# YuyangSunshine/ABR_IOD

Hardware: AMD Instinct MI355X
Metric: training images/sec (R50-C4 Faster R-CNN + ARD) (higher is better)
Workload: dtype f32 (tensors, accumulation and error bound; contractions via a 2-term fp16 split of both operands scaled by their amax, 3 cross products on the fp16 matrix cores: f16x3)

## Files before the change

abr_iod_amd/csrc/common.h:

```cpp
#pragma once
#include <hip/hip_runtime.h>
#include <stdint.h>
#include <stdio.h>

#include <functional>
#include <vector>

#include "abr_iod_hip.h"

namespace abr {

__device__ __forceinline__ float relu_f(const float v) { return v < 0.f ? 0.f : v; }


void set_error(const char* fmt, ...);

#define ABR_REQUIRE(cond, ...)                 \
    do {                                       \
        if (!(cond)) {                         \
            ::abr::set_error(__VA_ARGS__);     \
            return ABR_E_INVALID;              \
        }                                      \
    } while (0)

// ... 9 lines not shown
constexpr int kWave = 64;
constexpr int kNumXCD = 8;

__device__ __forceinline__ unsigned xcd_remap(unsigned bid, unsigned nblk) {
    const unsigned q = nblk / kNumXCD, r = nblk % kNumXCD;
    const unsigned xcd = bid % kNumXCD, pos = bid / kNumXCD;
    const unsigned base = xcd < r ? xcd * (q + 1) : r * (q + 1) + (xcd - r) * q;
    return base + pos;
}

__device__ __forceinline__ float wave_sum(float v) {
#pragma unroll
    for (int o = 32; o > 0; o >>= 1) v += __shfl_xor(v, o, 64);
    return v;
}
__device__ __forceinline__ float wave_max(float v) {
#pragma unroll
    for (int o = 32; o > 0; o >>= 1) v = fmaxf(v, __shfl_xor(v, o, 64));
    return v;
}

template <int NW>
__device__ __forceinline__ float block_sum(float v, float* sm) {
    v = wave_sum(v);
    const int w = threadIdx.x >> 6, l = threadIdx.x & 63;
    __syncthreads();
    if (l == 0) sm[w] = v;
    __syncthreads();
    float t = 0.f;
#pragma unroll
    for (int i = 0; i < NW; i++) t += sm[i];
    return t;
}

struct DetWs {
    float* part;
    unsigned* ticket;
};
DetWs det_ws(hipStream_t st, size_t nfloats);
template <int NV>
__device__ __forceinline__ bool det_sum_last(const float (&vals)[NV], const DetWs ws, float (&total)[NV]) {
    __shared__ int s_last;
    __shared__ float s_w[16];
    const unsigned nblk = gridDim.x * gridDim.y, bid = blockIdx.y * gridDim.x + blockIdx.x;
    if (threadIdx.x == 0) {
#pragma unroll
        for (int j = 0; j < NV; j++) __hip_atomic_store(ws.part + (size_t)bid * NV + j, vals[j], __ATOMIC_RELAXED, __HIP_MEMORY_SCOPE_AGENT);
        __builtin_amdgcn_fence(__ATOMIC_RELEASE, "agent");
        asm volatile("s_waitcnt vmcnt(0)" ::: "memory");
        s_last = atomicAdd(ws.ticket, 1u) == nblk - 1u;
    }
    __syncthreads();
    if (!s_last) return false;
    if (threadIdx.x == 0) {
        __builtin_amdgcn_fence(__ATOMIC_ACQUIRE, "agent");
        *ws.ticket = 0u;
    }
    __syncthreads();
#pragma unroll
    for (int j = 0; j < NV; j++) {
        float a = 0.f;
        for (unsigned i = threadIdx.x; i < nblk; i += blockDim.x) a += __hip_atomic_load(ws.part + (size_t)i * NV + j, __ATOMIC_RELAXED, __HIP_MEMORY_SCOPE_AGENT);
        a = wave_sum(a);
        __syncthreads();
        if ((threadIdx.x & 63) == 0) s_w[threadIdx.x >> 6] = a;
        __syncthreads();
        float t = 0.f;
        for (unsigned w = 0; w < (blockDim.x >> 6); w++) t += s_w[w];
        total[j] = t;
    }
    return true;
}

enum ProfId { PROF_IGEMM_128x128 = 0, PROF_IGEMM_128x64, PROF_IGEMM_64x64, PROF_IGEMM_SMALLC, PROF_WGRAD, PROF_ROIALIGN_FWD,
              PROF_ROIALIGN_BWD, PROF_IGEMM_BF16, PROF_WGRAD_BF16,
              PROF_X6_128x128, PROF_X6_128x64, PROF_X6_64x64, PROF_X6W_128x128, PROF_X6W_128x64, PROF_X6W_64x64, PROF_X6W_TAIL64,
              PROF_H3W_128x128, PROF_H3W_128x64, PROF_H3W_64x64, PROF_WGRAD_H3,
              PROF_F16W_128x128, PROF_F16W_128x64, PROF_F16W_64x64, PROF_WGRAD_F16, PROF_COUNT };
struct AmaxRef;
int wino_input_transform(const float* x, int B, int H, int W, int C, float* V, hipStream_t st, const AmaxRef* amax = nullptr);
int wino_output_transform(const float* M, int B, int H, int W, int N, const float* scale, const float* bias, int relu, const float* mask,
                          float* out, hipStream_t st, const AmaxRef* amax = nullptr);
int wino_outgrad_transform(const float* gy, int B, int H, int W, int N, float* Mg, hipStream_t st, const AmaxRef* amax = nullptr);
int wino_wgrad_inverse(const float* dU, int N, int C, const float* scale, float* dw, hipStream_t st);
float* wino_ws(hipStream_t st, size_t floats);
enum DerivedKind { DERIVED_NONE = -1, DERIVED_WINO_U = 0, DERIVED_X6_PLANES = 1, DERIVED_WINO_U_X6_PLANES = 2, DERIVED_H3_PLANES = 3, DERIVED_WINO_U_H3_PLANES = 4 };
void* derived_cached(const void* w, int kind, size_t bytes, int64_t version, hipStream_t st, const std::function<int(void*)>& fill);
void* derived_acquire(const void* w, int kind, size_t bytes, int64_t version, hipStream_t st, void** token, std::vector<hipStream_t>* waited = nullptr);
void derived_commit(void* const* tokens, int n, hipStream_t st);
void derived_abandon(void* const* tokens, int n);

struct ConvRoute {
    int math;
    int wgrad_math;
    bool fwd_wino;
    bool wgrad_wino;
    int64_t v_floats;
    int kind;
    int64_t rows;
    int K;
    size_t bytes;
};
ConvRoute conv_route(const abr_conv_desc& d);

struct PrepJob {
    const float* src;
    const float* scale;
    void* dst;
    int a, b, c;
    int gx, gy;
    int first_block;
};
struct PrepTable { const PrepJob* jobs; int njobs; };
template <int PrepJob::*F = &PrepJob::first_block>
__device__ __forceinline__ PrepJob prep_job(const PrepTable& t, int block) {
    int lo = 0, hi = t.njobs - 1;
    while (lo < hi) {
        const int mid = (lo + hi + 1) >> 1;
        if (t.jobs[mid].*F <= block) lo = mid; else hi = mid - 1;
    }
    return t.jobs[lo];
}
template <int PrepJob::*F = &PrepJob::first_block>
__device__ __forceinline__ PrepJob prep_job(const PrepJob& j, int) { return j; }
struct PrepJobs { int n = 0; PrepJob one{}; const PrepJob* dev = nullptr; };
template <class F>
void prep_each(const PrepJobs& s, F&& f) {
    if (s.n == 1) f(s.one);
    else if (s.n > 1) f(PrepTable{s.dev, s.n});
}
__device__ __forceinline__ size_t h3_planes_bytes_dev(int rows, int K) { return (size_t)((rows + 31) / 32 * 32) * (size_t)K * 4; }
__host__ __device__ __forceinline__ int prep_transpose_tile(int Cout, int Cin, const void* w, const void* wt) {
    return (((Cout | Cin) & 3) == 0 && ((reinterpret_cast<uintptr_t>(w) | reinterpret_cast<uintptr_t>(wt)) & 15) == 0) ? 64 : 32;
}
void prep_wino_u(const PrepJobs& jobs, int blocks, hipStream_t st);
void prep_wino_h3_direct(const PrepJobs& jobs, int pack_blocks, int scale_blocks, unsigned* flags, hipStream_t st);
void derived_cache_clear();
void derived_cache_drop_range(const void* base, size_t bytes);
size_t derived_cache_bytes();

unsigned* x6_flags_ptr();
constexpr unsigned kX6TinyB = (17u << 24) - 1u;
__device__ __forceinline__ void x6_report(unsigned bmin, float nonfin, unsigned* flags) {
    unsigned f = 0;
    if (bmin < kX6TinyB) f |= ABR_X6_FLAG_TINY;
    if (nonfin != nonfin) f |= ABR_X6_FLAG_NONFINITE;
    if (f) atomicOr(flags, f);
}

struct AmaxRef {
    unsigned long long* word;
    unsigned epoch;
};
constexpr unsigned kH3RangeBinades = 18;
AmaxRef h3_amax_alloc();
int h3_amax_reduce(const float* x, int64_t n, AmaxRef ref, hipStream_t st);
void h3_amax_remember(const void* tensor, AmaxRef ref);
AmaxRef h3_amax_recall(const void* tensor);

__device__ __forceinline__ unsigned h3_amax_load(const unsigned long long* word, unsigned epoch) {
    const unsigned long long v = __hip_atomic_load(word, __ATOMIC_RELAXED, __HIP_MEMORY_SCOPE_AGENT);
    return (unsigned)(v >> 32) == epoch ? (unsigned)v : 0xFFFFFFFFu;
}
__device__ __forceinline__ void h3_scales(unsigned amax_bits, float& s, float& inv_s) {
    int e = (int)(amax_bits >> 23);
    if (amax_bits == 0u || e >= 255) { s = 1.f; inv_s = 1.f; return; }
    e = e < 15 ? 15 : e;
// ... 84 lines not shown
```

abr_iod_amd/csrc/conv_wgrad.hip:

```cpp
#include <algorithm>

#include <map>
#include <mutex>

#include "common.h"

namespace {

typedef float f32x16 __attribute__((ext_vector_type(16)));
typedef _Float16 f16x8 __attribute__((ext_vector_type(8)));

constexpr int TN_ = 128;
constexpr int TK_ = 128;
constexpr int MR = 32;

struct FastDiv {
    unsigned mul, shr, d;
    __host__ void init(unsigned div) {
        d = div;
        shr = 0;
        while ((1u << shr) < div) shr++;
        mul = (unsigned)((((unsigned long long)1 << 32) * (((unsigned long long)1 << shr) - div)) / div + 1);
    }
    __device__ __forceinline__ void divmod(unsigned n, unsigned& q, unsigned& r) const {
        q = (__umulhi(n, mul) + n) >> shr;
        r = n - q * d;
    }
};

struct WgP {
    unsigned long long* prof_ts;
    int B, H, W, Cin, Cout, R, S, stride, pad, Ho, Wo;
    int M, K;
    int tiles_n, tiles_k, splits, mt_per_split;
    int plain;
    FastDiv d_howo, d_wo;
    const float* scale;
    unsigned x_bytes, gy_bytes;
    int overwrite;
    int nbatch, tiles_pb;
    long x_bs, gy_bs, dw_bs;
    int math;
    unsigned* x6_flags;
    float* ws;
    int final_store;
    int map4;
    const unsigned long long* gy_amax;
    const unsigned long long* x_amax;
    unsigned gy_epoch, x_epoch;
    unsigned long long* h3_stats;
};

__device__ __forceinline__ float2 wg_operand_scale(const WgP& p) {
    if (!p.gy_amax) return make_float2(1.f, 1.f);
    float sg, ig, sx, ix;
    abr::h3_scales(abr::h3_amax_load(p.gy_amax, p.gy_epoch), sg, ig);
    abr::h3_scales(abr::h3_amax_load(p.x_amax, p.x_epoch), sx, ix);
    return make_float2(sg, sx);
}

typedef f32x16 wg_f32x16;

constexpr unsigned kPartBytes = 16u * 256u * 16u;

__device__ __forceinline__ void wgrad_store_tile(const WgP& p, const float (&v)[4], int tm, int tn, int c, int n0, int k0, int wm, int wn, int l31, int lh,
                                                 bool store, float* __restrict__ dw, const float2 osc = make_float2(1.f, 1.f)) {
    const int k = p.map4 ? k0 + 4 * l31 + 2 * wn + tn : k0 + wn * 64 + 2 * l31 + tn;
    if (k >= p.K) return;
#pragma unroll
    for (int e = 0; e < 4; e++) {
        const int r = 4 * c + e;
        const int i = (r & 3) + 8 * (r >> 2) + 4 * lh;
        const int n = p.map4 ? n0 + 4 * i + 2 * wm + tm : n0 + wm * 64 + 2 * i + tm;
        if (n >= p.Cout) continue;
        const float sc = (p.scale ? p.scale[n] : 1.f) * fmaxf(osc.x, osc.y);
        const float val = (v[e] * fminf(osc.x, osc.y)) * sc;
        if (store) dw[(size_t)n * p.K + k] = val;
        else unsafeAtomicAdd(dw + (size_t)n * p.K + k, val);
    }
}

__device__ __forceinline__ void wgrad_finish(const WgP& p, f32x16 (&acc)[2][2], int n0, int k0, int wm, int wn, int l31, int lh, int tid,
                                             int gtile, int split, float* __restrict__ dw) {
    if (p.ws) {
        float4* dst = reinterpret_cast<float4*>(reinterpret_cast<char*>(p.ws) + ((size_t)gtile * p.splits + split) * kPartBytes) + tid;
#pragma unroll
        for (int t = 0; t < 4; t++)
#pragma unroll
            for (int c = 0; c < 4; c++) {
                const f32x16& a = acc[t >> 1][t & 1];
                dst[(t * 4 + c) * 256] = make_float4(a[4 * c], a[4 * c + 1], a[4 * c + 2], a[4 * c + 3]);
            }
        return;
    }
    const float2 osc = wg_operand_scale(p);
#pragma unroll
    for (int t = 0; t < 4; t++)
#pragma unroll
        for (int c = 0; c < 4; c++) {
            const f32x16& a = acc[t >> 1][t & 1];
            const float v[4] = {a[4 * c], a[4 * c + 1], a[4 * c + 2], a[4 * c + 3]};
            wgrad_store_tile(p, v, t >> 1, t & 1, c, n0, k0, wm, wn, l31, lh, p.overwrite != 0, dw, osc);
        }
}

__global__ __launch_bounds__(256) void wgrad_reduce_kernel(const WgP p, float* __restrict__ dw_) {
    const int gtile = blockIdx.x >> 4, quad = blockIdx.x & 15;
    const int tid = threadIdx.x, lane = tid & 63, wave = tid >> 6;
    const float4* src = reinterpret_cast<const float4*>(reinterpret_cast<const char*>(p.ws) + (size_t)gtile * p.splits * kPartBytes) + quad * 256 + tid;
    float4 sum = make_float4(0.f, 0.f, 0.f, 0.f);
    int q = 0;
    for (; q + 4 <= p.splits; q += 4) {
        const float4 v0 = src[(size_t)q * (kPartBytes / 16)], v1 = src[(size_t)(q + 1) * (kPartBytes / 16)];
        const float4 v2 = src[(size_t)(q + 2) * (kPartBytes / 16)], v3 = src[(size_t)(q + 3) * (kPartBytes / 16)];
        sum.x += v0.x; sum.y += v0.y; sum.z += v0.z; sum.w += v0.w;
        sum.x += v1.x; sum.y += v1.y; sum.z += v1.z; sum.w += v1.w;
        sum.x += v2.x; sum.y += v2.y; sum.z += v2.z; sum.w += v2.w;
        sum.x += v3.x; sum.y += v3.y; sum.z += v3.z; sum.w += v3.w;
    }
    for (; q < p.splits; q++) {
        const float4 v = src[(size_t)q * (kPartBytes / 16)];
        sum.x += v.x; sum.y += v.y; sum.z += v.z; sum.w += v.w;
    }
    float* dw = dw_;
    int tile = gtile;
    if (p.nbatch > 1) {
        const int bt = tile / p.tiles_pb;
        tile -= bt * p.tiles_pb;
        dw += bt * p.dw_bs;
    }
    const int n0 = (tile % p.tiles_n) * TN_, k0 = (tile / p.tiles_n) * TK_;
    const float v[4] = {sum.x, sum.y, sum.z, sum.w};
    const int t = quad >> 2, c = quad & 3;
    wgrad_store_tile(p, v, t >> 1, t & 1, c, n0, k0, wave >> 1, wave & 1, lane & 31, lane >> 5, p.final_store != 0, dw, wg_operand_scale(p));
}

template <bool SB>
__global__ __launch_bounds__(256) void conv_wgrad_kernel(const WgP p, const float* __restrict__ x_,
                                                          const float* __restrict__ gy_, float* __restrict__ dw_) {
    const float* x = x_;
    const float* gy = gy_;
    float* dw = dw_;
    extern __shared__ __attribute__((aligned(16))) float smem[];
    static_assert(SB, "single-buffered only");
    abr::prof_stamp_begin(p.prof_ts);
    float* Gs = smem;
    float* As = smem + MR * TN_;

    const unsigned bid = abr::xcd_remap(blockIdx.x, gridDim.x);
    const int total_tiles = p.tiles_pb * (p.nbatch > 1 ? p.nbatch : 1);
    const int split = bid / total_tiles;
    int tile = bid % total_tiles;
    const int gtile = tile;
    if (p.nbatch > 1) {
        const int bt = tile / p.tiles_pb;
        tile -= bt * p.tiles_pb;
        x += bt * p.x_bs; gy += bt * p.gy_bs; dw += bt * p.dw_bs;
    }
    const int tile_n = tile % p.tiles_n, tile_k = tile / p.tiles_n;
    const int n0 = tile_n * TN_, k0 = tile_k * TK_;
    const int tid = threadIdx.x, lane = tid & 63, wave = tid >> 6;
    const int wm = wave >> 1, wn = wave & 1;

    const int q = tid & 31, r8 = tid >> 5;
    const int gn = n0 + q * 4;
    const bool g_ok = gn < p.Cout;
    const int ak = k0 + q * 4;
    const bool k_ok = ak < p.K;
    int fr = 0, fs = 0, fc = 0;
    if (k_ok) {
        const int rs = ak / p.Cin;
        fc = ak % p.Cin;
        fr = rs / p.S;
        fs = rs % p.S;
    }
    const int mt0 = split * p.mt_per_split;
    const int mt1 = min(mt0 + p.mt_per_split, (p.M + MR - 1) / MR);

    constexpr unsigned kOOB = 0x80000000u;
    const __amdgpu_buffer_rsrc_t rgy = __builtin_amdgcn_make_buffer_rsrc(const_cast<float*>(gy), 0, p.gy_bytes, 0x00020000);
    const __amdgpu_buffer_rsrc_t rxx = __builtin_amdgcn_make_buffer_rsrc(const_cast<float*>(x), 0, p.x_bytes, 0x00020000);
    const unsigned g_voff = g_ok ? (unsigned)(r8 * p.Cout + gn) * 4u : kOOB;
    const unsigned a_voff_plain = k_ok ? (unsigned)(r8 * p.Cin + fc) * 4u : kOOB;
    const int a_const = ((fr - p.pad) * p.W + (fs - p.pad)) * p.Cin + fc;
    float4 rg[4], ra[4];
    auto fetch = [&](__amdgpu_buffer_rsrc_t r, unsigned voff, int soff) -> float4 {
        typedef unsigned u32x4 __attribute__((ext_vector_type(4)));
        const u32x4 v = __builtin_amdgcn_raw_buffer_load_b128(r, (int)voff, soff, 0);
        return make_float4(__uint_as_float(v.x), __uint_as_float(v.y), __uint_as_float(v.z), __uint_as_float(v.w));
    };
    auto load_tile = [&](int mt) {
#pragma unroll
        for (int i = 0; i < 4; i++) {
            const int mrow = mt * MR + 8 * i;
            rg[i] = fetch(rgy, g_voff + (unsigned)(mrow * p.Cout) * 4u, 0);
            if (p.plain) {
                ra[i] = fetch(rxx, a_voff_plain + (unsigned)(mrow * p.Cin) * 4u, 0);
            } else {
                const int m = mrow + r8;
                unsigned b, rem, ho, wo;
                p.d_howo.divmod((unsigned)m, b, rem);
                p.d_wo.divmod(rem, ho, wo);
                const int hi = (int)ho * p.stride - p.pad + fr, wi = (int)wo * p.stride - p.pad + fs;
                const bool ok = k_ok & (m < p.M) & ((unsigned)hi < (unsigned)p.H) & ((unsigned)wi < (unsigned)p.W);
                const int off = (((int)b * p.H + (int)ho * p.stride) * p.W + (int)wo * p.stride) * p.Cin + a_const;
                ra[i] = fetch(rxx, ok ? (unsigned)off * 4u : kOOB, 0);
            }
        }
    };
    auto store_tile = [&]() {
#pragma unroll
        for (int i = 0; i < 4; i++) {
            *reinterpret_cast<float4*>(Gs + (r8 + 8 * i) * TN_ + q * 4) = rg[i];
            *reinterpret_cast<float4*>(As + (r8 + 8 * i) * TK_ + q * 4) = ra[i];
        }
    };

// ... 195 lines not shown
                *reinterpret_cast<u32x4*>(st_base + j * 128 + PL) = o1;
                *reinterpret_cast<u32x4*>(st_base + j * 128 + 2 * PL) = o2;
            }
        }
    };

    f32x16 acc[2][2];
#pragma unroll
    for (int i = 0; i < 2; i++)
#pragma unroll
        for (int j = 0; j < 2; j++)
#pragma unroll
            for (int r = 0; r < 16; r++) acc[i][j][r] = 0.f;

    const int l31 = lane & 31, lh = lane >> 5;
    const unsigned* const g_rd = Gs + ((lh * 4 + 2 * wm) * 32 + l31) * 4;
    const unsigned* const a_rd = As + ((lh * 4 + 2 * wn) * 32 + l31) * 4;
    auto compute_tile = [&]() {
#pragma unroll
        for (int s = 0; s < MRX / 16; s++) {
            bf16x8 G[2][NPL], A[2][NPL];
#pragma unroll
            for (int pl = 0; pl < NPL; pl++)
#pragma unroll
                for (int t = 0; t < 2; t++) {
                    G[t][pl] = *reinterpret_cast<const bf16x8*>(g_rd + pl * PL + (s * 8 + t) * 128);
                    A[t][pl] = *reinterpret_cast<const bf16x8*>(a_rd + pl * PL + (s * 8 + t) * 128);
                }
            constexpr int pg[6] = {NP == 1 ? 0 : (H3 ? 1 : 2), 0, H3 ? 0 : 1, 1, 0, 0}, pa[6] = {0, NP == 1 ? 0 : (H3 ? 1 : 2), H3 ? 0 : 1, 0, 1, 0};
#pragma unroll
            for (int t = 0; t < NP; t++)
#pragma unroll
                for (int i = 0; i < 2; i++)
#pragma unroll
                    for (int j = 0; j < 2; j++) {
                        if constexpr (HF) acc[i][j] = __builtin_amdgcn_mfma_f32_32x32x16_f16(__builtin_bit_cast(f16x8, G[i][pg[t]]), __builtin_bit_cast(f16x8, A[j][pa[t]]), acc[i][j], 0, 0, 0);
                        else acc[i][j] = __builtin_amdgcn_mfma_f32_32x32x16_bf16(G[i][pg[t]], A[j][pa[t]], acc[i][j], 0, 0, 0);
                    }
        }
    };
    if (mt0 < mt1) {
        load_tile(mt0);
        store_tile();
        __syncthreads();
        int mt = mt0;
        for (; mt + 1 < mt1; mt++) {
            load_tile(mt + 1);
            __builtin_amdgcn_sched_barrier(0);
            compute_tile();
            __syncthreads();
            store_tile();
            __syncthreads();
        }
        compute_tile();
    }
    if constexpr (HF) {
        if (chk) abr::h3_report(op_bits, nsmall, p.x6_flags, p.h3_stats);
    } else {
        if (chk) abr::x6_report(bmin, nonfin, p.x6_flags);
    }

    wgrad_finish(p, acc, n0, k0, wm, wn, l31, lh, tid, gtile, split, dw);
    abr::prof_stamp_end(p.prof_ts);
}

}

static float* wgrad_scratch(hipStream_t st, size_t units) {
    struct Ws { float* ws = nullptr; size_t units = 0; };
    static std::map<hipStream_t, Ws> pool;
    static std::mutex mu;
    std::lock_guard<std::mutex> g(mu);
    Ws& w = pool[st];
    if (w.units < units) {
        if (w.ws) { (void)hipStreamSynchronize(st); (void)hipFree(w.ws); w.ws = nullptr; w.units = 0; }
        if (hipMalloc(&w.ws, units * 65536) != hipSuccess) return nullptr;
        w.units = units;
    }
    return w.ws;
}

static void wgrad_plan_reduction(WgP& p, int tiles, hipStream_t st) {
    p.ws = nullptr;
    if (p.splits <= 1) { if (p.final_store) p.overwrite = 1; return; }
    p.ws = wgrad_scratch(st, (size_t)tiles * p.splits);
}

static void wgrad_reduce(const WgP& p, int tiles, float* dw, hipStream_t st) {
    if (p.ws) wgrad_reduce_kernel<<<(unsigned)tiles * 16u, 256, 0, st>>>(p, dw);
}

static void launch_wgrad(WgP p, const float* x, const float* gy, float* dw, void* stream) {
    const int nb = p.nbatch > 1 ? p.nbatch : 1;
    p.tiles_pb = p.tiles_n * p.tiles_k;
    const int m_tiles = (p.M + MR - 1) / MR;
    int32_t info[3];
    const int cus = abr_device_info(info) == ABR_OK ? info[0] : 256;
    const int tiles = p.tiles_n * p.tiles_k * nb;
    const int max_splits = std::max(1, (m_tiles + 7) / 8);
    int splits = 1;
    double best = -1.0;
    for (int sp = 1; sp <= max_splits; sp++) {
        const long wgs = (long)tiles * sp;
        if (wgs > 8L * cus && sp > 1) break;
        const long rounds = (wgs + cus - 1) / cus;
        double eff = (double)wgs / (double)(rounds * cus);
        if (wgs < cus) eff *= 0.5;
        else if (wgs < 2L * cus && m_tiles / (2 * sp) >= 64) eff *= 0.85;
        eff -= 0.0002 * sp;
        if (eff > best) { best = eff; splits = sp; }
    }
    if (p.overwrite) splits = 1;
    p.splits = splits;
    p.mt_per_split = (m_tiles + splits - 1) / splits;
    wgrad_plan_reduction(p, tiles, abr::as_stream(stream));
    if (p.final_store && splits > 1 && !p.ws) {
        (void)hipMemsetAsync(dw, 0, sizeof(float) * (size_t)nb * p.Cout * p.K, abr::as_stream(stream));
        p.final_store = 0;
    }
    if (p.math == ABR_MATH_BF16X6 || p.math == ABR_MATH_BF16 || p.math == ABR_MATH_F16X3 || p.math == ABR_MATH_F16) {
        static bool attr6 = false;
        const bool one = p.math == ABR_MATH_BF16;
        const bool h3 = p.math == ABR_MATH_F16X3;
        const bool f16 = p.math == ABR_MATH_F16;
        const size_t lds6 = sizeof(unsigned) * (one || f16 ? 1 : (h3 ? 2 : 3)) * (MRX / 2) * (TN_ + TK_);
        if (!attr6) {
            (void)hipFuncSetAttribute(reinterpret_cast<const void*>(conv_wgrad_x6_kernel<6>), hipFuncAttributeMaxDynamicSharedMemorySize,
                                      (int)(sizeof(unsigned) * 3 * (MRX / 2) * (TN_ + TK_)));
            attr6 = true;
        }
        p.map4 = 1;
        p.x6_flags = !one ? abr::x6_flags_ptr() : nullptr;
        p.h3_stats = (h3 && p.x6_flags) ? abr::h3_stats_ptr() : nullptr;
        if (p.h3_stats) abr::h3_stats_inspected((double)nb * p.M * ((double)p.Cout + (double)p.K));
        const int pid6 = h3 ? abr::PROF_WGRAD_H3 : (f16 ? abr::PROF_WGRAD_F16 : abr::PROF_WGRAD_BF16);
        const int rec6 = abr::prof_start(abr::as_stream(stream), pid6, 2.0 * (double)p.M * (double)p.Cout * (double)p.K * nb);
        p.prof_ts = abr::prof_clock_slot(rec6);
        abr::prof_add_bytes(pid6, 4.0 * nb * ((double)p.M * p.Cout + (p.plain ? (double)p.M * p.K : (double)p.B * p.H * p.W * p.Cin) + (double)p.Cout * p.K));
        if (h3) conv_wgrad_x6_kernel<3><<<(unsigned)(tiles * splits), 256, lds6, abr::as_stream(stream)>>>(p, x, gy, dw);
        else if (f16) conv_wgrad_x6_kernel<1, true><<<(unsigned)(tiles * splits), 256, lds6, abr::as_stream(stream)>>>(p, x, gy, dw);
        else if (one) conv_wgrad_x6_kernel<1><<<(unsigned)(tiles * splits), 256, lds6, abr::as_stream(stream)>>>(p, x, gy, dw);
        else conv_wgrad_x6_kernel<6><<<(unsigned)(tiles * splits), 256, lds6, abr::as_stream(stream)>>>(p, x, gy, dw);
        abr::prof_stop(abr::as_stream(stream), rec6);
        wgrad_reduce(p, tiles, dw, abr::as_stream(stream));
        return;
    }
    const int rec = abr::prof_start(abr::as_stream(stream), abr::PROF_WGRAD, 2.0 * (double)p.M * (double)p.Cout * (double)p.K * nb);
    p.prof_ts = abr::prof_clock_slot(rec);
    conv_wgrad_kernel<true><<<(unsigned)(tiles * splits), 256, sizeof(float) * MR * (TN_ + TK_), abr::as_stream(stream)>>>(p, x, gy, dw);
    abr::prof_stop(abr::as_stream(stream), rec);
    wgrad_reduce(p, tiles, dw, abr::as_stream(stream));
}

extern "C" int abr_conv_wgrad(const abr_conv_desc* d, const float* x, const float* gy, float* dw, void* stream) {
    ABR_REQUIRE(d && x && gy && dw, "conv_wgrad: null pointer");
    ABR_REQUIRE(d->Cin % 4 == 0 && d->Cout % 4 == 0, "conv_wgrad: Cin and Cout must be multiples of 4");
    ABR_REQUIRE(d->Ho == (d->H + 2 * d->pad - d->R) / d->stride + 1 && d->Wo == (d->W + 2 * d->pad - d->S) / d->stride + 1,
                "conv_wgrad: Ho/Wo inconsistent");
    WgP p;
    p.B = d->B; p.H = d->H; p.W = d->W; p.Cin = d->Cin; p.Cout = d->Cout; p.R = d->R; p.S = d->S;
    p.stride = d->stride; p.pad = d->pad; p.Ho = d->Ho; p.Wo = d->Wo;
    p.M = d->B * d->Ho * d->Wo;
    p.K = d->R * d->S * d->Cin;
    p.plain = (d->R == 1 && d->S == 1 && d->stride == 1 && d->pad == 0);
    p.scale = d->scale;
    const int64_t xb = (int64_t)d->B * d->H * d->W * d->Cin * 4, gb = (int64_t)p.M * d->Cout * 4;
    ABR_REQUIRE(xb < (int64_t)0x7FFFFFF0 && gb < (int64_t)0x7FFFFFF0, "conv_wgrad: activation / gradient tensors must be < 2 GB (32-bit buffer offsets)");
    p.x_bytes = (unsigned)xb; p.gy_bytes = (unsigned)gb;
    p.d_howo.init((unsigned)(d->Ho * d->Wo)); p.d_wo.init((unsigned)d->Wo);
    p.tiles_n = (p.Cout + TN_ - 1) / TN_;
    p.tiles_k = (p.K + TK_ - 1) / TK_;
    if (p.M == 0) return ABR_OK;
    p.nbatch = 1; p.tiles_pb = 0; p.x_bs = p.gy_bs = p.dw_bs = 0; p.overwrite = 0;
    p.ws = nullptr; p.final_store = 0; p.map4 = 0;
    p.x6_flags = nullptr;
    p.gy_amax = p.x_amax = nullptr; p.gy_epoch = p.x_epoch = 0; p.h3_stats = nullptr;
    hipStream_t st = abr::as_stream(stream);
    ABR_REQUIRE(d->math == ABR_MATH_F32 || d->math == ABR_MATH_BF16 || d->math == ABR_MATH_BF16X6 || d->math == ABR_MATH_F16X3 || d->math == ABR_MATH_F16,
                "conv_wgrad: unknown math mode");
    const abr::ConvRoute route = abr::conv_route(*d);
    p.math = route.wgrad_math;
    const bool h3 = p.math == ABR_MATH_F16X3 || p.math == ABR_MATH_F16;
    abr::AmaxRef gy_ref{reinterpret_cast<unsigned long long*>(const_cast<uint64_t*>(d->gy_amax)), d->gy_amax_epoch};
    abr::AmaxRef x_ref{reinterpret_cast<unsigned long long*>(const_cast<uint64_t*>(d->x_amax)), d->x_amax_epoch};
    auto need_ref = [&](abr::AmaxRef& r, const float* t, int64_t n) -> bool {
        if (r.word) return true;
        r = abr::h3_amax_alloc();
        return r.word && abr::h3_amax_reduce(t, n, r, st) == 0;
    };
    if (route.wgrad_wino) {
        const int th_n = (d->H + 3) / 4, tw_n = (d->W + 3) / 4;
        const int64_t T = (int64_t)d->B * th_n * tw_n;
        const size_t nV = (size_t)36 * T * d->Cin, nM = (size_t)36 * T * d->Cout, nU = (size_t)36 * d->Cout * d->Cin;
        float* vin = route.v_floats ? d->wino_v : nullptr;
        float* ws = abr::wino_ws(st, (vin ? 0 : nV) + nM + nU);
        if (ws) {
            float* V = vin ? vin : ws;
            float *Mg = ws + (vin ? 0 : nV), *dU = Mg + nM;
            abr::AmaxRef v_ref{nullptr, 0}, m_ref{nullptr, 0};
            if (h3) {
                if (vin) v_ref = abr::h3_amax_recall(vin);
                else v_ref = abr::h3_amax_alloc();
                m_ref = abr::h3_amax_alloc();
                ABR_REQUIRE(m_ref.word && (vin || v_ref.word), "conv_wgrad (f16x3): no amax words");
                if (vin && !v_ref.word) ABR_REQUIRE(need_ref(v_ref, vin, (int64_t)nV), "conv_wgrad (f16x3): amax reduction failed");
            }
            int bad = vin ? 0 : abr::wino_input_transform(x, d->B, d->H, d->W, d->Cin, V, st, h3 ? &v_ref : nullptr);
            bad |= abr::wino_outgrad_transform(gy, d->B, d->H, d->W, d->Cout, Mg, st, h3 ? &m_ref : nullptr);
            int32_t info[3];
            const int cus_ = abr_device_info(info) == ABR_OK ? info[0] : 256;
            const long out_tiles = 36L * ((d->Cout + TN_ - 1) / TN_) * ((d->Cin + TK_ - 1) / TK_);
            const int own = out_tiles >= 2L * cus_;
            if (!bad) {
                WgP g = p;
                g.overwrite = own;
                g.final_store = !own;
                g.B = (int)T; g.H = g.W = 1; g.R = g.S = 1; g.stride = 1; g.pad = 0; g.Ho = g.Wo = 1;
                g.M = (int)T; g.K = d->Cin; g.plain = 1; g.scale = nullptr;
                g.d_howo.init(1u); g.d_wo.init(1u);
                g.tiles_n = (g.Cout + TN_ - 1) / TN_; g.tiles_k = (g.K + TK_ - 1) / TK_;
                g.x_bytes = (unsigned)(T * d->Cin * 4); g.gy_bytes = (unsigned)(T * d->Cout * 4);
                g.nbatch = 36; g.x_bs = (long)T * d->Cin; g.gy_bs = (long)T * d->Cout; g.dw_bs = (long)d->Cout * d->Cin;
                if (h3) { g.x_amax = v_ref.word; g.x_epoch = v_ref.epoch; g.gy_amax = m_ref.word; g.gy_epoch = m_ref.epoch; }
                launch_wgrad(g, V, Mg, dU, stream);
                bad = abr::wino_wgrad_inverse(dU, d->Cout, d->Cin, d->scale, dw, st);
            }
            ABR_REQUIRE(!bad, "conv_wgrad: winograd launch failed");
            ABR_CHECK_LAUNCH("conv_wgrad (winograd)");
            return ABR_OK;
        }
    }
    if (h3) {
        ABR_REQUIRE(need_ref(gy_ref, gy, (int64_t)p.M * d->Cout) && need_ref(x_ref, x, (int64_t)d->B * d->H * d->W * d->Cin), "conv_wgrad (f16x3): amax reduction failed");
        p.gy_amax = gy_ref.word; p.gy_epoch = gy_ref.epoch; p.x_amax = x_ref.word; p.x_epoch = x_ref.epoch;
    }
    launch_wgrad(p, x, gy, dw, stream);
    ABR_CHECK_LAUNCH("conv_wgrad");
    return ABR_OK;
}
```

abr_iod_amd/csrc/conv_winograd.hip:

```cpp
#include <map>

#include <algorithm>
#include <map>
#include <functional>
#include <mutex>
#include <utility>
#include <type_traits>
#include <vector>

#include "common.h"

namespace {

template <int V>
struct vf {
    float v[V];
};
template <int V>
__device__ __forceinline__ vf<V> operator+(vf<V> a, vf<V> b) {
    vf<V> r;
#pragma unroll
    for (int i = 0; i < V; i++) r.v[i] = a.v[i] + b.v[i];
    return r;
}
// ... 323 lines not shown
#pragma unroll
                for (int j = 0; j < 4; j++) {
                    const int oy = 4 * th + i, ox = 4 * tw + j;
                    const bool in = oy < H && ox < W;
                    mk[i][j] = vld<V>(mask + (((int64_t)b * H + (in ? oy : 4 * th)) * W + (in ? ox : 4 * tw)) * N + n);
                }
        }
#pragma unroll
        for (int i = 0; i < 4; i++) {
            f2 y[4];
            at4(tcol[i][0], tcol[i][1], tcol[i][2], tcol[i][3], tcol[i][4], tcol[i][5], y[0], y[1], y[2], y[3]);
            const int oy = 4 * th + i;
            if (oy >= H) continue;
#pragma unroll
            for (int j = 0; j < 4; j++) {
                const int ox = 4 * tw + j;
                if (ox >= W) continue;
                const int64_t o = (((int64_t)b * H + oy) * W + ox) * N + n;
                f2 v;
#pragma unroll
                for (int e = 0; e < V; e++) {
                    v.v[e] = y[j].v[e] * sc.v[e] + bi.v[e];
                    if (relu) v.v[e] = abr::relu_f(v.v[e]);
                }
                if (mask) {
#pragma unroll
                    for (int e = 0; e < V; e++) v.v[e] = mk[i][j].v[e] > 0.f ? v.v[e] : 0.f;
                }
                vst(out + o, v);
                if (amax) am = vabs_max(am, v);
            }
        }
    }
    if (amax) abr::h3_amax_emit(amax, epoch, am);
}

template <typename T>
__device__ __forceinline__ void a6(const T y0, const T y1, const T y2, const T y3, T& o0, T& o1, T& o2, T& o3, T& o4, T& o5) {
    o0 = y0;
    o1 = y0 + y1 + y2 + y3;
    o2 = y0 - y1 + y2 - y3;
    o3 = y0 + 2.f * y1 + 4.f * y2 + 8.f * y3;
    o4 = y0 - 2.f * y1 + 4.f * y2 - 8.f * y3;
    o5 = y3;
}

template <int V>
__global__ __launch_bounds__(256) void wino_outgrad_kernel(const float* __restrict__ gy, int B, int H, int W, int N, int th_n, int tw_n,
                                                           float* __restrict__ Mg, unsigned long long* amax, unsigned epoch) {
    typedef vf<V> f2;
    unsigned am = 0;
    const int64_t T = (int64_t)B * th_n * tw_n;
    const int N2 = N / V;
    const int64_t total = T * N2;
    const int64_t ps = T * N;
    for (int64_t idx = (int64_t)blockIdx.x * blockDim.x + threadIdx.x; idx < total; idx += (int64_t)gridDim.x * blockDim.x) {
        const int n = V * (int)(idx % N2);
        const int64_t t = idx / N2;
        const int tw = (int)(t % tw_n), th = (int)((t / tw_n) % th_n), b = (int)(t / ((int64_t)tw_n * th_n));
        f2 tcol[6][4];
#pragma unroll
        for (int j = 0; j < 4; j++) {
            const int ox = 4 * tw + j;
            f2 y[4];
#pragma unroll
            for (int i = 0; i < 4; i++) {
                const int oy = 4 * th + i;
                y[i] = (oy < H && ox < W) ? vld<V>(gy + (((int64_t)b * H + oy) * W + ox) * N + n) : vzero<V>();
            }
            a6(y[0], y[1], y[2], y[3], tcol[0][j], tcol[1][j], tcol[2][j], tcol[3][j], tcol[4][j], tcol[5][j]);
        }
#pragma unroll
        for (int i = 0; i < 6; i++) {
            f2 v0, v1, v2, v3, v4, v5;
            a6(tcol[i][0], tcol[i][1], tcol[i][2], tcol[i][3], v0, v1, v2, v3, v4, v5);
            float* o = Mg + ((int64_t)(6 * i) * T + t) * N + n;
            vst(o, v0); vst(o + ps, v1); vst(o + 2 * ps, v2); vst(o + 3 * ps, v3); vst(o + 4 * ps, v4); vst(o + 5 * ps, v5);
            if (amax) am = vabs_max(vabs_max(vabs_max(vabs_max(vabs_max(vabs_max(am, v0), v1), v2), v3), v4), v5);
        }
    }
    if (amax) abr::h3_amax_emit(amax, epoch, am);
}

template <typename T>
__device__ __forceinline__ void gt3(const T u0, const T u1, const T u2, const T u3, const T u4, const T u5, T& o0, T& o1, T& o2) {
    o0 = 0.25f * u0 - (1.f / 6.f) * (u1 + u2) + (1.f / 24.f) * (u3 + u4);
    o1 = (1.f / 6.f) * (u2 - u1) + (1.f / 12.f) * (u3 - u4);
    o2 = (1.f / 6.f) * (u3 + u4 - u1 - u2) + u5;
}

template <int V>
__global__ __launch_bounds__(256) void wino_wgrad_inverse_kernel(const float* __restrict__ dU, int N, int C, const float* __restrict__ scale,
                                                                 float* __restrict__ dw) {
    typedef vf<V> fv;
    const int Cv = C / V;
    const int64_t total = (int64_t)N * Cv;
    const int64_t ps = (int64_t)N * C;
    for (int64_t idx = (int64_t)blockIdx.x * blockDim.x + threadIdx.x; idx < total; idx += (int64_t)gridDim.x * blockDim.x) {
        const int c = V * (int)(idx % Cv);
        const int64_t n = idx / Cv;
        const float* u = dU + n * C + c;
        fv tcol[3][6];
#pragma unroll
        for (int j = 0; j < 6; j++)
            gt3(vld<V>(u + (0 + j) * ps), vld<V>(u + (6 + j) * ps), vld<V>(u + (12 + j) * ps), vld<V>(u + (18 + j) * ps), vld<V>(u + (24 + j) * ps),
                vld<V>(u + (30 + j) * ps), tcol[0][j], tcol[1][j], tcol[2][j]);
        const float sc = scale ? scale[n] : 1.f;
        fv old[3][3];
#pragma unroll
        for (int r = 0; r < 3; r++)
#pragma unroll
            for (int q = 0; q < 3; q++) old[r][q] = vld<V>(dw + ((n * 3 + r) * 3 + q) * C + c);
#pragma unroll
        for (int r = 0; r < 3; r++) {
            fv g0, g1, g2;
            gt3(tcol[r][0], tcol[r][1], tcol[r][2], tcol[r][3], tcol[r][4], tcol[r][5], g0, g1, g2);
            float* o = dw + ((n * 3 + r) * 3) * C + c;
            vst(o, old[r][0] + sc * g0); vst(o + C, old[r][1] + sc * g1); vst(o + 2 * C, old[r][2] + sc * g2);
        }
    }
}

inline unsigned grid_for(int64_t n) { return (unsigned)std::min<int64_t>((n + 255) / 256, 32768); }
inline unsigned grid_for(int64_t n, bool) { return grid_for(n); }

}

namespace abr {

static inline bool wide(int64_t tiles, int C) {
    return C % 4 == 0 && tiles * (C / 4) >= (int64_t)256 * 4 * 256;
}

int wino_input_transform(const float* x, int B, int H, int W, int C, float* V, hipStream_t st, const AmaxRef* amax) {
    const int th_n = (H + 3) / 4, tw_n = (W + 3) / 4;
    unsigned long long* aw = amax ? amax->word : nullptr;
    const unsigned ae = amax ? amax->epoch : 0u;
    wino_input_kernel<2><<<grid_for((int64_t)B * th_n * tw_n * (C / 2), aw != nullptr), 256, 0, st>>>(x, B, H, W, C, th_n, tw_n, V, aw, ae);
    return hipGetLastError() == hipSuccess ? 0 : 1;
}

void prep_wino_h3_direct(const PrepJobs& jobs, int pack_blocks, int scale_blocks, unsigned* flags, hipStream_t st) {
    if (!jobs.n) return;
    static std::once_flag attr_once;
    std::call_once(attr_once, [] {
        (void)hipFuncSetAttribute(reinterpret_cast<const void*>(wino_h3_pack_multi_kernel<PrepTable>), hipFuncAttributeMaxDynamicSharedMemorySize, (int)kWhLds);
        (void)hipFuncSetAttribute(reinterpret_cast<const void*>(wino_h3_pack_multi_kernel<PrepJob>), hipFuncAttributeMaxDynamicSharedMemorySize, (int)kWhLds);
    });
    prep_each(jobs, [&](auto src) {
        wino_h3_scales_multi_kernel<<<(unsigned)scale_blocks, 256, 0, st>>>(src, flags);
        wino_h3_pack_multi_kernel<<<(unsigned)pack_blocks, 256, kWhLds, st>>>(src);
    });
}

void prep_wino_u(const PrepJobs& jobs, int blocks, hipStream_t st) {
    prep_each(jobs, [&](auto src) { wino_weight_multi_kernel<<<(unsigned)blocks, 256, 0, st>>>(src); });
}

int wino_output_transform(const float* Mm, int B, int H, int W, int N, const float* scale, const float* bias, int relu, const float* mask,
                          float* out, hipStream_t st, const AmaxRef* amax) {
    const int th_n = (H + 3) / 4, tw_n = (W + 3) / 4;
    unsigned long long* aw = amax ? amax->word : nullptr;
    const unsigned ae = amax ? amax->epoch : 0u;
    if (wide((int64_t)B * th_n * tw_n, N))
        wino_output_kernel<4><<<grid_for((int64_t)B * th_n * tw_n * (N / 4), aw != nullptr), 256, 0, st>>>(Mm, B, H, W, N, th_n, tw_n, scale, bias, relu, mask, out, aw, ae);
    else
        wino_output_kernel<2><<<grid_for((int64_t)B * th_n * tw_n * (N / 2), aw != nullptr), 256, 0, st>>>(Mm, B, H, W, N, th_n, tw_n, scale, bias, relu, mask, out, aw, ae);
    return hipGetLastError() == hipSuccess ? 0 : 1;
}

int wino_outgrad_transform(const float* gy, int B, int H, int W, int N, float* Mg, hipStream_t st, const AmaxRef* amax) {
    const int th_n = (H + 3) / 4, tw_n = (W + 3) / 4;
    unsigned long long* aw = amax ? amax->word : nullptr;
    const unsigned ae = amax ? amax->epoch : 0u;
    if (wide((int64_t)B * th_n * tw_n, N)) wino_outgrad_kernel<4><<<grid_for((int64_t)B * th_n * tw_n * (N / 4), aw != nullptr), 256, 0, st>>>(gy, B, H, W, N, th_n, tw_n, Mg, aw, ae);
    else wino_outgrad_kernel<2><<<grid_for((int64_t)B * th_n * tw_n * (N / 2), aw != nullptr), 256, 0, st>>>(gy, B, H, W, N, th_n, tw_n, Mg, aw, ae);
    return hipGetLastError() == hipSuccess ? 0 : 1;
}

int wino_wgrad_inverse(const float* dU, int N, int C, const float* scale, float* dw, hipStream_t st) {
    if (C % 4 == 0) wino_wgrad_inverse_kernel<4><<<grid_for((int64_t)N * (C / 4)), 256, 0, st>>>(dU, N, C, scale, dw);
    else wino_wgrad_inverse_kernel<2><<<grid_for((int64_t)N * (C / 2)), 256, 0, st>>>(dU, N, C, scale, dw);
    return hipGetLastError() == hipSuccess ? 0 : 1;
}

float* wino_ws(hipStream_t st, size_t floats) {
    struct Ws { float* buf = nullptr; size_t floats = 0; };
    static std::map<hipStream_t, Ws> pool;
    static std::mutex mu;
    std::lock_guard<std::mutex> g(mu);
    Ws& w = pool[st];
    if (w.floats < floats) {
        if (w.buf) { (void)hipStreamSynchronize(st); (void)hipFree(w.buf); w.buf = nullptr; w.floats = 0; }
        if (hipMalloc(&w.buf, floats * sizeof(float)) != hipSuccess) return nullptr;
        w.floats = floats;
    }
    return w.buf;
}

namespace {
struct DEntry {
    void* buf = nullptr; size_t bytes = 0; int64_t version = 0; hipStream_t stream = nullptr; hipEvent_t filled = nullptr;
    std::vector<hipStream_t> readers;
    uint64_t last_use = 0;
    int64_t pending = 0;
};
std::map<std::pair<const void*, int>, DEntry> g_dcache;
std::mutex g_dcache_mu;
uint64_t g_dcache_clock = 0;
size_t g_dcache_bytes = 0;

void dcache_drop(DEntry& e) {
    if (e.stream) (void)hipStreamSynchronize(e.stream);
    for (hipStream_t r : e.readers) (void)hipStreamSynchronize(r);
    if (e.buf) { (void)hipFree(e.buf); g_dcache_bytes -= e.bytes; }
    if (e.filled) (void)hipEventDestroy(e.filled);
    e = DEntry();
}
size_t dcache_limit() {
    static const size_t mb = getenv("ABR_WINO_CACHE_MB") ? (size_t)atoll(getenv("ABR_WINO_CACHE_MB")) : 4096;
    return mb << 20;
}
}

static DEntry* dcache_acquire_locked(const void* w, int kind, size_t bytes, int64_t version, hipStream_t st, bool* needs_fill, std::vector<hipStream_t>* waited = nullptr) {
    DEntry& e = g_dcache[std::make_pair(w, kind)];
    e.last_use = ++g_dcache_clock;
    if (e.buf && e.bytes != bytes) dcache_drop(e);
    if (!e.buf) {
        while (g_dcache_bytes + bytes > dcache_limit()) {
            auto victim = g_dcache.end();
            for (auto it = g_dcache.begin(); it != g_dcache.end(); ++it)
                if (it->second.buf && &it->second != &e && !it->second.pending && (victim == g_dcache.end() || it->second.last_use < victim->second.last_use)) victim = it;
            if (victim == g_dcache.end()) break;
            dcache_drop(victim->second);
            g_dcache.erase(victim);
        }
        if (hipMalloc(&e.buf, bytes) != hipSuccess) { e.buf = nullptr; return nullptr; }
        e.bytes = bytes;
        g_dcache_bytes += bytes;
        e.last_use = g_dcache_clock;
        if (!e.filled) (void)hipEventCreateWithFlags(&e.filled, hipEventDisableTiming);
    }
    if (e.version == version && !e.pending) {
        if (st != e.stream && std::find(e.readers.begin(), e.readers.end(), st) == e.readers.end()) {
            (void)hipStreamWaitEvent(st, e.filled, 0);
            e.readers.push_back(st);
        }
        *needs_fill = false;
        return &e;
    }
    std::vector<hipStream_t> users = e.readers;
    if (e.stream && e.stream != st) users.push_back(e.stream);
    for (hipStream_t r : users) {
        if (r == st) continue;
        if (waited) {
            if (std::find(waited->begin(), waited->end(), r) != waited->end()) continue;
            waited->push_back(r);
        }
        hipEvent_t ev = nullptr;
        if (hipEventCreateWithFlags(&ev, hipEventDisableTiming) != hipSuccess) { (void)hipStreamSynchronize(r); continue; }
        (void)hipEventRecord(ev, r);
        (void)hipStreamWaitEvent(st, ev, 0);
        (void)hipEventDestroy(ev);
    }
// ... 81 lines not shown
```

Before: 224.2.

## Fuse Winograd wgrad split reduction with inverse transform into one finish kernel

For the Winograd weight-gradient path, the batched 36-plane GEMM now always writes partials to scratch. A new finish kernel sums the splits, applies the operand scales and performs the G^T dU G inverse transform through shared memory, accumulating directly into dw. This removes the intermediate dU buffer, the separate reduce and inverse-transform launches and the extra global round trip. The cost is that scratch is now required even when there is a single split, and the launch fails if scratch cannot be obtained.

```diff
diff --git a/abr_iod_amd/csrc/common.h b/abr_iod_amd/csrc/common.h
--- a/abr_iod_amd/csrc/common.h
+++ b/abr_iod_amd/csrc/common.h
@@ -115,7 +115,6 @@
 int wino_output_transform(const float* M, int B, int H, int W, int N, const float* scale, const float* bias, int relu, const float* mask,
                           float* out, hipStream_t st, const AmaxRef* amax = nullptr);
 int wino_outgrad_transform(const float* gy, int B, int H, int W, int N, float* Mg, hipStream_t st, const AmaxRef* amax = nullptr);
-int wino_wgrad_inverse(const float* dU, int N, int C, const float* scale, float* dw, hipStream_t st);
 float* wino_ws(hipStream_t st, size_t floats);
 enum DerivedKind { DERIVED_NONE = -1, DERIVED_WINO_U = 0, DERIVED_X6_PLANES = 1, DERIVED_WINO_U_X6_PLANES = 2, DERIVED_H3_PLANES = 3, DERIVED_WINO_U_H3_PLANES = 4 };
 void* derived_cached(const void* w, int kind, size_t bytes, int64_t version, hipStream_t st, const std::function<int(void*)>& fill);
diff --git a/abr_iod_amd/csrc/conv_wgrad.hip b/abr_iod_amd/csrc/conv_wgrad.hip
--- a/abr_iod_amd/csrc/conv_wgrad.hip
+++ b/abr_iod_amd/csrc/conv_wgrad.hip
@@ -43,7 +43,7 @@
     int math;
     unsigned* x6_flags;
     float* ws;
-    int final_store;
+    int one_split;
     int map4;
     const unsigned long long* gy_amax;
     const unsigned long long* x_amax;
@@ -104,10 +104,10 @@
         }
 }
 
-__global__ __launch_bounds__(256) void wgrad_reduce_kernel(const WgP p, float* __restrict__ dw_) {
-    const int gtile = blockIdx.x >> 4, quad = blockIdx.x & 15;
+__global__ __launch_bounds__(256) void wgrad_reduce_kernel(const WgP p, float* __restrict__ dw) {
+    const int tile = blockIdx.x >> 4, quad = blockIdx.x & 15;
     const int tid = threadIdx.x, lane = tid & 63, wave = tid >> 6;
-    const float4* src = reinterpret_cast<const float4*>(reinterpret_cast<const char*>(p.ws) + (size_t)gtile * p.splits * kPartBytes) + quad * 256 + tid;
+    const float4* src = reinterpret_cast<const float4*>(reinterpret_cast<const char*>(p.ws) + (size_t)tile * p.splits * kPartBytes) + quad * 256 + tid;
     float4 sum = make_float4(0.f, 0.f, 0.f, 0.f);
     int q = 0;
     for (; q + 4 <= p.splits; q += 4) {
@@ -122,17 +122,108 @@
         const float4 v = src[(size_t)q * (kPartBytes / 16)];
         sum.x += v.x; sum.y += v.y; sum.z += v.z; sum.w += v.w;
     }
-    float* dw = dw_;
-    int tile = gtile;
-    if (p.nbatch > 1) {
-        const int bt = tile / p.tiles_pb;
-        tile -= bt * p.tiles_pb;
-        dw += bt * p.dw_bs;
-    }
     const int n0 = (tile % p.tiles_n) * TN_, k0 = (tile / p.tiles_n) * TK_;
     const float v[4] = {sum.x, sum.y, sum.z, sum.w};
     const int t = quad >> 2, c = quad & 3;
-    wgrad_store_tile(p, v, t >> 1, t & 1, c, n0, k0, wave >> 1, wave & 1, lane & 31, lane >> 5, p.final_store != 0, dw, wg_operand_scale(p));
+    wgrad_store_tile(p, v, t >> 1, t & 1, c, n0, k0, wave >> 1, wave & 1, lane & 31, lane >> 5, false, dw, wg_operand_scale(p));
+}
+
+struct WgSlot {
+    int nl, kl;
+    unsigned off[4];
+};
+__device__ __forceinline__ WgSlot wgrad_slot(int map4, int slot) {
+    const int lane = slot & 63, w = slot >> 6;
+    const int e = lane & 3, kq = (lane >> 2) | ((w & 1) << 4);
+    const int tm = (w >> 1) & 1, wm = (w >> 2) & 1, lh = (w >> 3) & 1, c = w >> 4;
+    const int i = e + 8 * c + 4 * lh;
+    WgSlot s;
+    s.nl = map4 ? 4 * i + 2 * wm + tm : wm * 64 + 2 * i + tm;
+    s.kl = 4 * kq;
+#pragma unroll
+    for (int kk = 0; kk < 4; kk++) {
+        const int tn = kk & 1;
+        const int wn = map4 ? kk >> 1 : kq >> 4;
+        const int l31 = map4 ? kq : 2 * (kq & 15) + (kk >> 1);
+        s.off[kk] = (unsigned)(((tm * 2 + tn) * 4 + c) * 1024 + ((wm * 2 + wn) * 64 + lh * 32 + l31) * 4 + e);
+    }
+    return s;
+}
+
+struct f4 {
+    float v[4];
+};
+__device__ __forceinline__ void gt3(const f4& u0, const f4& u1, const f4& u2, const f4& u3, const f4& u4, const f4& u5, f4& o0, f4& o1, f4& o2) {
+#pragma clang fp contract(off)
+    constexpr float k6 = 1.f / 6.f, k12 = 1.f / 12.f, k24 = 1.f / 24.f;
+#pragma unroll
+    for (int c = 0; c < 4; c++) {
+        o0.v[c] = fmaf(u3.v[c] + u4.v[c], k24, fmaf(u0.v[c], 0.25f, -((u1.v[c] + u2.v[c]) * k6)));
+        o1.v[c] = (c & 1) ? fmaf(u2.v[c] - u1.v[c], k6, (u3.v[c] - u4.v[c]) * k12) : fmaf(u3.v[c] - u4.v[c], k12, (u2.v[c] - u1.v[c]) * k6);
+        o2.v[c] = fmaf(((u3.v[c] + u4.v[c]) - u1.v[c]) - u2.v[c], k6, u5.v[c]);
+    }
+}
+
+constexpr int kFinSlots = 64;
+__global__ __launch_bounds__(6 * kFinSlots) void wino_wgrad_finish_kernel(const WgP p, const float* __restrict__ scale, float* __restrict__ dw) {
+#pragma clang fp contract(off)
+    __shared__ float4 tcol[6][3][kFinSlots];
+    const int tile = blockIdx.x / (4096 / kFinSlots), sl = threadIdx.x & (kFinSlots - 1), j = threadIdx.x / kFinSlots;
+    const WgSlot s = wgrad_slot(p.map4, (blockIdx.x % (4096 / kFinSlots)) * kFinSlots + sl);
+    const int n = (tile % p.tiles_n) * TN_ + s.nl, k = (tile / p.tiles_n) * TK_ + s.kl;
+    const bool inside = n < p.Cout && k < p.K;
+    const float2 osc = wg_operand_scale(p);
+    const float lo = fminf(osc.x, osc.y), hi = 1.f * fmaxf(osc.x, osc.y);
+    const size_t unit = (size_t)p.splits * (kPartBytes / 4), batch = (size_t)p.tiles_pb * unit;
+    const float* src = p.ws + (size_t)tile * unit + (size_t)j * batch;
+    if (inside) {
+        f4 u[6];
+#pragma unroll
+        for (int i = 0; i < 6; i++)
+#pragma unroll
+            for (int kk = 0; kk < 4; kk++) u[i].v[kk] = src[(size_t)(6 * i) * batch + s.off[kk]];
+        if (p.splits > 1) {
+#pragma unroll
+            for (int i = 0; i < 6; i++)
+#pragma unroll
+                for (int kk = 0; kk < 4; kk++) u[i].v[kk] = 0.f + u[i].v[kk];
+            for (int q = 1; q < p.splits; q++) {
+#pragma unroll
+                for (int i = 0; i < 6; i++)
+#pragma unroll
+                    for (int kk = 0; kk < 4; kk++) u[i].v[kk] += src[(size_t)(6 * i) * batch + (size_t)q * (kPartBytes / 4) + s.off[kk]];
+            }
+        }
+#pragma unroll
+        for (int i = 0; i < 6; i++)
+#pragma unroll
+            for (int kk = 0; kk < 4; kk++) u[i].v[kk] = (u[i].v[kk] * lo) * hi;
+        f4 t[3];
+        gt3(u[0], u[1], u[2], u[3], u[4], u[5], t[0], t[1], t[2]);
+#pragma unroll
+        for (int r = 0; r < 3; r++) tcol[j][r][sl] = make_float4(t[r].v[0], t[r].v[1], t[r].v[2], t[r].v[3]);
+    }
+    __syncthreads();
+    if (!inside || j >= 3) return;
+    const int r = j;
+    float4* o = reinterpret_cast<float4*>(dw + ((size_t)n * 3 + r) * 3 * p.K + k);
+    const int pitch = p.K / 4;
+    const float4 old[3] = {o[0], o[pitch], o[2 * pitch]};
+    const float sc = scale ? scale[n] : 1.f;
+    f4 c[6], g[3];
+#pragma unroll
+    for (int jj = 0; jj < 6; jj++) {
+        const float4 v = tcol[jj][r][sl];
+        c[jj] = {{v.x, v.y, v.z, v.w}};
+    }
+    gt3(c[0], c[1], c[2], c[3], c[4], c[5], g[0], g[1], g[2]);
+#pragma unroll
+    for (int q = 0; q < 3; q++) {
+        typedef float f32x4 __attribute__((ext_vector_type(4)));
+        f32x4 v = {fmaf(sc, g[q].v[0], old[q].x), fmaf(sc, g[q].v[1], old[q].y), fmaf(sc, g[q].v[2], old[q].z), fmaf(sc, g[q].v[3], old[q].w)};
+        asm volatile("" : "+v"(v));
+        *reinterpret_cast<f32x4*>(o + q * pitch) = v;
+    }
 }
 
 template <bool SB>
@@ -494,15 +585,17 @@
 
 static void wgrad_plan_reduction(WgP& p, int tiles, hipStream_t st) {
     p.ws = nullptr;
-    if (p.splits <= 1) { if (p.final_store) p.overwrite = 1; return; }
+    if (p.splits <= 1 && p.nbatch <= 1) return;
     p.ws = wgrad_scratch(st, (size_t)tiles * p.splits);
 }
 
-static void wgrad_reduce(const WgP& p, int tiles, float* dw, hipStream_t st) {
-    if (p.ws) wgrad_reduce_kernel<<<(unsigned)tiles * 16u, 256, 0, st>>>(p, dw);
-}
-
-static void launch_wgrad(WgP p, const float* x, const float* gy, float* dw, void* stream) {
+static void wgrad_reduce(const WgP& p, int tiles, const float* wino_scale, float* dw, hipStream_t st) {
+    if (!p.ws) return;
+    if (p.nbatch > 1) wino_wgrad_finish_kernel<<<(unsigned)p.tiles_pb * (4096u / kFinSlots), 6 * kFinSlots, 0, st>>>(p, wino_scale, dw);
+    else wgrad_reduce_kernel<<<(unsigned)tiles * 16u, 256, 0, st>>>(p, dw);
+}
+
+static bool launch_wgrad(WgP p, const float* x, const float* gy, float* dw, void* stream, const float* wino_scale = nullptr) {
     const int nb = p.nbatch > 1 ? p.nbatch : 1;
     p.tiles_pb = p.tiles_n * p.tiles_k;
     const int m_tiles = (p.M + MR - 1) / MR;
@@ -522,14 +615,11 @@
         eff -= 0.0002 * sp;
         if (eff > best) { best = eff; splits = sp; }
     }
-    if (p.overwrite) splits = 1;
+    if (p.one_split) splits = 1;
     p.splits = splits;
     p.mt_per_split = (m_tiles + splits - 1) / splits;
     wgrad_plan_reduction(p, tiles, abr::as_stream(stream));
-    if (p.final_store && splits > 1 && !p.ws) {
-        (void)hipMemsetAsync(dw, 0, sizeof(float) * (size_t)nb * p.Cout * p.K, abr::as_stream(stream));
-        p.final_store = 0;
-    }
+    if (nb > 1 && !p.ws) return false;
     if (p.math == ABR_MATH_BF16X6 || p.math == ABR_MATH_BF16 || p.math == ABR_MATH_F16X3 || p.math == ABR_MATH_F16) {
         static bool attr6 = false;
         const bool one = p.math == ABR_MATH_BF16;
@@ -554,14 +644,15 @@
         else if (one) conv_wgrad_x6_kernel<1><<<(unsigned)(tiles * splits), 256, lds6, abr::as_stream(stream)>>>(p, x, gy, dw);
         else conv_wgrad_x6_kernel<6><<<(unsigned)(tiles * splits), 256, lds6, abr::as_stream(stream)>>>(p, x, gy, dw);
         abr::prof_stop(abr::as_stream(stream), rec6);
-        wgrad_reduce(p, tiles, dw, abr::as_stream(stream));
-        return;
+        wgrad_reduce(p, tiles, wino_scale, dw, abr::as_stream(stream));
+        return true;
     }
     const int rec = abr::prof_start(abr::as_stream(stream), abr::PROF_WGRAD, 2.0 * (double)p.M * (double)p.Cout * (double)p.K * nb);
     p.prof_ts = abr::prof_clock_slot(rec);
     conv_wgrad_kernel<true><<<(unsigned)(tiles * splits), 256, sizeof(float) * MR * (TN_ + TK_), abr::as_stream(stream)>>>(p, x, gy, dw);
     abr::prof_stop(abr::as_stream(stream), rec);
-    wgrad_reduce(p, tiles, dw, abr::as_stream(stream));
+    wgrad_reduce(p, tiles, wino_scale, dw, abr::as_stream(stream));
+    return true;
 }
 
 extern "C" int abr_conv_wgrad(const abr_conv_desc* d, const float* x, const float* gy, float* dw, void* stream) {
@@ -584,7 +675,7 @@
     p.tiles_k = (p.K + TK_ - 1) / TK_;
     if (p.M == 0) return ABR_OK;
     p.nbatch = 1; p.tiles_pb = 0; p.x_bs = p.gy_bs = p.dw_bs = 0; p.overwrite = 0;
-    p.ws = nullptr; p.final_store = 0; p.map4 = 0;
+    p.ws = nullptr; p.one_split = 0; p.map4 = 0;
     p.x6_flags = nullptr;
     p.gy_amax = p.x_amax = nullptr; p.gy_epoch = p.x_epoch = 0; p.h3_stats = nullptr;
     hipStream_t st = abr::as_stream(stream);
@@ -603,12 +694,12 @@
     if (route.wgrad_wino) {
         const int th_n = (d->H + 3) / 4, tw_n = (d->W + 3) / 4;
         const int64_t T = (int64_t)d->B * th_n * tw_n;
-        const size_t nV = (size_t)36 * T * d->Cin, nM = (size_t)36 * T * d->Cout, nU = (size_t)36 * d->Cout * d->Cin;
+        const size_t nV = (size_t)36 * T * d->Cin, nM = (size_t)36 * T * d->Cout;
         float* vin = route.v_floats ? d->wino_v : nullptr;
-        float* ws = abr::wino_ws(st, (vin ? 0 : nV) + nM + nU);
+        float* ws = abr::wino_ws(st, (vin ? 0 : nV) + nM);
         if (ws) {
             float* V = vin ? vin : ws;
-            float *Mg = ws + (vin ? 0 : nV), *dU = Mg + nM;
+            float* Mg = ws + (vin ? 0 : nV);
             abr::AmaxRef v_ref{nullptr, 0}, m_ref{nullptr, 0};
             if (h3) {
                 if (vin) v_ref = abr::h3_amax_recall(vin);
@@ -625,8 +716,7 @@
             const int own = out_tiles >= 2L * cus_;
             if (!bad) {
                 WgP g = p;
-                g.overwrite = own;
-                g.final_store = !own;
+                g.one_split = own;
                 g.B = (int)T; g.H = g.W = 1; g.R = g.S = 1; g.stride = 1; g.pad = 0; g.Ho = g.Wo = 1;
                 g.M = (int)T; g.K = d->Cin; g.plain = 1; g.scale = nullptr;
                 g.d_howo.init(1u); g.d_wo.init(1u);
@@ -634,8 +724,7 @@
                 g.x_bytes = (unsigned)(T * d->Cin * 4); g.gy_bytes = (unsigned)(T * d->Cout * 4);
                 g.nbatch = 36; g.x_bs = (long)T * d->Cin; g.gy_bs = (long)T * d->Cout; g.dw_bs = (long)d->Cout * d->Cin;
                 if (h3) { g.x_amax = v_ref.word; g.x_epoch = v_ref.epoch; g.gy_amax = m_ref.word; g.gy_epoch = m_ref.epoch; }
-                launch_wgrad(g, V, Mg, dU, stream);
-                bad = abr::wino_wgrad_inverse(dU, d->Cout, d->Cin, d->scale, dw, st);
+                bad = !launch_wgrad(g, V, Mg, dw, stream, d->scale);
             }
             ABR_REQUIRE(!bad, "conv_wgrad: winograd launch failed");
             ABR_CHECK_LAUNCH("conv_wgrad (winograd)");
diff --git a/abr_iod_amd/csrc/conv_winograd.hip b/abr_iod_amd/csrc/conv_winograd.hip
--- a/abr_iod_amd/csrc/conv_winograd.hip
+++ b/abr_iod_amd/csrc/conv_winograd.hip
@@ -429,45 +429,6 @@
     if (amax) abr::h3_amax_emit(amax, epoch, am);
 }
 
-template <typename T>
-__device__ __forceinline__ void gt3(const T u0, const T u1, const T u2, const T u3, const T u4, const T u5, T& o0, T& o1, T& o2) {
-    o0 = 0.25f * u0 - (1.f / 6.f) * (u1 + u2) + (1.f / 24.f) * (u3 + u4);
-    o1 = (1.f / 6.f) * (u2 - u1) + (1.f / 12.f) * (u3 - u4);
-    o2 = (1.f / 6.f) * (u3 + u4 - u1 - u2) + u5;
-}
-
-template <int V>
-__global__ __launch_bounds__(256) void wino_wgrad_inverse_kernel(const float* __restrict__ dU, int N, int C, const float* __restrict__ scale,
-                                                                 float* __restrict__ dw) {
-    typedef vf<V> fv;
-    const int Cv = C / V;
-    const int64_t total = (int64_t)N * Cv;
-    const int64_t ps = (int64_t)N * C;
-    for (int64_t idx = (int64_t)blockIdx.x * blockDim.x + threadIdx.x; idx < total; idx += (int64_t)gridDim.x * blockDim.x) {
-        const int c = V * (int)(idx % Cv);
-        const int64_t n = idx / Cv;
-        const float* u = dU + n * C + c;
-        fv tcol[3][6];
-#pragma unroll
-        for (int j = 0; j < 6; j++)
-            gt3(vld<V>(u + (0 + j) * ps), vld<V>(u + (6 + j) * ps), vld<V>(u + (12 + j) * ps), vld<V>(u + (18 + j) * ps), vld<V>(u + (24 + j) * ps),
-                vld<V>(u + (30 + j) * ps), tcol[0][j], tcol[1][j], tcol[2][j]);
-        const float sc = scale ? scale[n] : 1.f;
-        fv old[3][3];
-#pragma unroll
-        for (int r = 0; r < 3; r++)
-#pragma unroll
-            for (int q = 0; q < 3; q++) old[r][q] = vld<V>(dw + ((n * 3 + r) * 3 + q) * C + c);
-#pragma unroll
-        for (int r = 0; r < 3; r++) {
-            fv g0, g1, g2;
-            gt3(tcol[r][0], tcol[r][1], tcol[r][2], tcol[r][3], tcol[r][4], tcol[r][5], g0, g1, g2);
-            float* o = dw + ((n * 3 + r) * 3) * C + c;
-            vst(o, old[r][0] + sc * g0); vst(o + C, old[r][1] + sc * g1); vst(o + 2 * C, old[r][2] + sc * g2);
-        }
-    }
-}
-
 inline unsigned grid_for(int64_t n) { return (unsigned)std::min<int64_t>((n + 255) / 256, 32768); }
 inline unsigned grid_for(int64_t n, bool) { return grid_for(n); }
 
@@ -522,12 +483,6 @@
     const unsigned ae = amax ? amax->epoch : 0u;
     if (wide((int64_t)B * th_n * tw_n, N)) wino_outgrad_kernel<4><<<grid_for((int64_t)B * th_n * tw_n * (N / 4), aw != nullptr), 256, 0, st>>>(gy, B, H, W, N, th_n, tw_n, Mg, aw, ae);
     else wino_outgrad_kernel<2><<<grid_for((int64_t)B * th_n * tw_n * (N / 2), aw != nullptr), 256, 0, st>>>(gy, B, H, W, N, th_n, tw_n, Mg, aw, ae);
-    return hipGetLastError() == hipSuccess ? 0 : 1;
-}
-
-int wino_wgrad_inverse(const float* dU, int N, int C, const float* scale, float* dw, hipStream_t st) {
-    if (C % 4 == 0) wino_wgrad_inverse_kernel<4><<<grid_for((int64_t)N * (C / 4)), 256, 0, st>>>(dU, N, C, scale, dw);
-    else wino_wgrad_inverse_kernel<2><<<grid_for((int64_t)N * (C / 2)), 256, 0, st>>>(dU, N, C, scale, dw);
     return hipGetLastError() == hipSuccess ? 0 : 1;
 }
 
```

New measurement: 225.7, median of 6. Within noise of the previous version (+0.7%).
